# hieucnm/GNN-RecSys

Measured on AMD Instinct MI355X. Metric: edges aggregated/sec, full-graph embed pass, d=128, higher is better.
Workload: dtype fp32

## Files before the change

### gnn-recsys_amd/csrc/spmm_project.hip

```cpp
#include "common.hpp"
#include "gather.hpp"
#include "rowq.hpp"
#include <cstdlib>
#include <type_traits>

namespace gnnrec {
namespace {

constexpr int kPD = 128;
constexpr int kPWaves = 16;
constexpr int kPRows = 2;
constexpr int kFusedChunk = 8;

struct EpiArgs {
  bool relu, l2, attn;
  int accum;
  float out_div, a0, a1;
  float* attn_state;
  float* out;
  int64_t ldo;
  int j0;
};

__device__ __forceinline__ void epilogue_row(const EpiArgs& e, int64_t row, bool valid,
                                             float y0, float y1) {
  activate(e.relu, e.l2, y0, y1);
  float keep = 0.f, nrm_attn = 1.f;
  if (e.attn) {
    float sc = y0 * e.a0 + y1 * e.a1;
#pragma unroll
    for (int off = 1; off < 64; off <<= 1) sc += __shfl_xor(sc, off);
    float mnew = sc, snew = 1.f, cnew = 1.f;
    if (valid && e.accum != GNNREC_ACC_ATTN_FIRST) {
      const float2 st = reinterpret_cast<const float2*>(e.attn_state)[row];
      mnew = fmaxf(st.x, sc);
      keep = expf(st.x - mnew);
      cnew = expf(sc - mnew);
      snew = st.y * keep + cnew;
    }
    if (e.accum == GNNREC_ACC_ATTN_LAST) nrm_attn = 1.f / snew;
    if (valid && (threadIdx.x & 63) == 0)
      reinterpret_cast<float2*>(e.attn_state)[row] = make_float2(mnew, snew);
    y0 *= cnew;
    y1 *= cnew;
  }
  if (!valid) return;
  float2* p = reinterpret_cast<float2*>(e.out + row * e.ldo + e.j0);
  if (e.attn) {
    if (e.accum != GNNREC_ACC_ATTN_FIRST) {
      const float2 o = *p;
      y0 = o.x * keep + y0;
      y1 = o.y * keep + y1;
    }
    y0 *= nrm_attn;
    y1 *= nrm_attn;
  } else if (e.accum != GNNREC_ACC_STORE) {
    const float2 o = *p;
    if (e.accum == GNNREC_ACC_ADD) {
      y0 = o.x + y0;
      y1 = o.y + y1;
    } else {
      y0 = fmaxf(o.x, y0);
      y1 = fmaxf(o.y, y1);
    }
  }
  if (e.out_div > 0.f) {
    y0 = y0 / e.out_div;
    y1 = y1 / e.out_div;
  }
  st_stream2(reinterpret_cast<float*>(p), y0, y1);
}

constexpr int kAggNone = GNNREC_AGG_NONE, kAggSave = GNNREC_AGG_SAVE, kAggLoad = GNNREC_AGG_LOAD;

template <int REDUCE, bool WEIGHTED, int UNROLL, int AGG = kAggNone>
__global__ __launch_bounds__(kPWaves * 64) void spmm_project_kernel(
    const int64_t* __restrict__ indptr, const int32_t* __restrict__ indices,
    const float* __restrict__ ew, const float* __restrict__ X, int64_t ldx,
    const float* __restrict__ H, int64_t ldh, const float* __restrict__ WsT,
    const float* __restrict__ WnT, const float* __restrict__ bias,
    const float* __restrict__ bias_ne, int64_t n_dst, int epilogue, int accum, float out_div,
    const float* __restrict__ attn_vec, float* __restrict__ attn_state,
    float* __restrict__ out, int64_t ldo, unsigned* rq, int rq_ch, float* __restrict__ agg,
    int64_t lda) {
  __shared__ float Ws[kPD * kPD];
  __shared__ float Wn[kPD * kPD];
  __shared__ float slots[kPWaves][kPRows][2][kPD];
  for (int i = threadIdx.x; i < kPD * kPD / 4; i += kPWaves * 64) {
    reinterpret_cast<float4*>(Ws)[i] = reinterpret_cast<const float4*>(WsT)[i];
    reinterpret_cast<float4*>(Wn)[i] = reinterpret_cast<const float4*>(WnT)[i];
  }
  __syncthreads();

  constexpr int LPR = 32, VEC = 4;
  const int lane = threadIdx.x & 63, wave = threadIdx.x >> 6;
  const int grp = lane / LPR;
  const int col = (lane % LPR) * VEC;
  const int j0 = 2 * lane;
  const bool relu = epilogue & GNNREC_EPI_RELU;
  const bool l2 = epilogue & GNNREC_EPI_L2NORM;
  const float init = (REDUCE == GNNREC_REDUCE_MAX) ? -INFINITY : 0.f;
  const int64_t stride = (int64_t)gridDim.x * kPWaves * kPRows;
  const float b0 = bias ? bias[j0] : 0.f, b1 = bias ? bias[j0 + 1] : 0.f;
  const float c0 = bias_ne ? bias_ne[j0] : 0.f, c1 = bias_ne ? bias_ne[j0 + 1] : 0.f;
  const bool attn = accum >= GNNREC_ACC_ATTN_FIRST;
  const float a0 = attn ? attn_vec[j0] : 0.f, a1 = attn ? attn_vec[j0 + 1] : 0.f;
  const EpiArgs ep{relu, l2, attn, accum, out_div, a0, a1, attn_state, out, ldo, j0};

  auto step = [&](int64_t row0, int64_t lim) {
    bool nonempty[kPRows];
    const int nv = (int)(lim - row0 < kPRows ? lim - row0 : kPRows);
    const int64_t ipl = lane <= nv ? ld_stream(indptr + row0 + lane) : 0;
    int64_t rb[kPRows + 1];
#pragma unroll
    for (int r = 0; r <= kPRows; ++r) rb[r] = __shfl(ipl, r <= nv ? r : nv);
    int pidx[kPRows];
    float4 hsr[kPRows];
#pragma unroll
    for (int r = 0; r < kPRows; ++r) {
      const bool valid = r < nv;
      hsr[r] = make_float4(0.f, 0.f, 0.f, 0.f);
      if constexpr (AGG == kAggLoad) {
        pidx[r] = 0;
        if (valid) hsr[r] = ld_stream4((grp == 0 ? agg + (row0 + r) * lda
                                                 : H + (row0 + r) * ldh) + col);
      } else {
        pidx[r] = valid && lane < rb[r + 1] - rb[r] ? ld_stream(indices + rb[r] + lane) : 0;
        if (valid && grp == 1) hsr[r] = ld_stream4(H + (row0 + r) * ldh + col);
      }
    }
#pragma unroll
    for (int r = 0; r < kPRows; ++r) {
      const bool valid = r < nv;
      const float4 hs = hsr[r];
      if constexpr (AGG == kAggLoad) {
        nonempty[r] = rb[r + 1] - rb[r] > 0;
        *reinterpret_cast<float4*>(&slots[wave][r][grp][col]) = hs;
        continue;
      }
      Frag<VEC> acc;
#pragma unroll
      for (int v = 0; v < VEC; ++v) acc.v[v] = init;
      int64_t deg = 0;
      if (valid) {
        const int64_t beg = rb[r], end = rb[r + 1];
        deg = end - beg;
        gather_range<LPR, VEC, REDUCE, WEIGHTED, UNROLL, true>(beg, end, indices, ew, X, ldx,
                                                               col, true, lane, grp, acc, pidx[r]);
      }
      combine_groups<LPR, VEC, REDUCE>(acc);
      finalize<VEC, REDUCE>(acc, deg, 0);
      nonempty[r] = deg > 0;
      if (grp == 0) {
        *reinterpret_cast<float4*>(&slots[wave][r][0][col]) =
            make_float4(acc.v[0], acc.v[1], acc.v[2], acc.v[3]);
        if constexpr (AGG == kAggSave)
          if (valid) store_frag<VEC>(agg + (row0 + r) * lda + col, acc);
      } else {
        *reinterpret_cast<float4*>(&slots[wave][r][1][col]) = hs;
      }
    }
    asm volatile("s_waitcnt lgkmcnt(0)" ::: "memory");

    float z[kPRows][2];
#pragma unroll
    for (int r = 0; r < kPRows; ++r) {
      z[r][0] = b0 + (nonempty[r] ? c0 : 0.f);
      z[r][1] = b1 + (nonempty[r] ? c1 : 0.f);
    }
#pragma unroll 2
    for (int k = 0; k < kPD; k += 4) {
      float4 a4[kPRows], s4[kPRows];
#pragma unroll
      for (int r = 0; r < kPRows; ++r) {
        a4[r] = *reinterpret_cast<const float4*>(&slots[wave][r][0][k]);
        s4[r] = *reinterpret_cast<const float4*>(&slots[wave][r][1][k]);
      }
#pragma unroll
      for (int kk = 0; kk < 4; ++kk) {
        const float2 ws = *reinterpret_cast<const float2*>(&Ws[(k + kk) * kPD + j0]);
        const float2 wn = *reinterpret_cast<const float2*>(&Wn[(k + kk) * kPD + j0]);
#pragma unroll
        for (int r = 0; r < kPRows; ++r) {
          const float s = kk == 0 ? s4[r].x : kk == 1 ? s4[r].y : kk == 2 ? s4[r].z : s4[r].w;
          const float a = kk == 0 ? a4[r].x : kk == 1 ? a4[r].y : kk == 2 ? a4[r].z : a4[r].w;
          z[r][0] = fmaf(s, ws.x, z[r][0]);
          z[r][0] = fmaf(a, wn.x, z[r][0]);
          z[r][1] = fmaf(s, ws.y, z[r][1]);
          z[r][1] = fmaf(a, wn.y, z[r][1]);
        }
      }
    }
    asm volatile("s_waitcnt lgkmcnt(0)" ::: "memory");

#pragma unroll
    for (int r = 0; r < kPRows; ++r) epilogue_row(ep, row0 + r, row0 + r < lim, z[r][0], z[r][1]);
  };

  if (rq != nullptr) {
    rq_for_each(rq, n_dst, rq_ch, [&](int64_t r0, int64_t r1) {
      for (int64_t row0 = r0; row0 < r1; row0 += kPRows) step(row0, r1);
    });
    rq_finish(rq);
    return;
  }
  for (int64_t row0 = ((int64_t)blockIdx.x * kPWaves + wave) * kPRows; row0 < n_dst;
       row0 += stride)
    step(row0, n_dst);
}


constexpr int kSppU = 4;
constexpr int kSpmU = 4;
constexpr int kSpmLU = 2;
constexpr int kSpmEU = 4;
constexpr int kMT = 32;
constexpr int kMWaves = 8;
constexpr int kMRows = kMT / kMWaves;
constexpr int kALd = 2 * kPD + 4;
constexpr int kCLd = kPD + 8;
constexpr int kALds = kMT * kALd;
static_assert(kMRows == 4, "a wave gathers its rows with one gather_lockstep4");

template <int REDUCE, bool WEIGHTED, int UNROLL, bool PRE>
__global__ __launch_bounds__(kMWaves * 64, 4) void spmm_project_mfma_kernel(
    const int64_t* __restrict__ indptr, const int32_t* __restrict__ indices,
    const float* __restrict__ ew, const float* __restrict__ X, int64_t ldx,
    const float* __restrict__ H, int64_t ldh, const float* __restrict__ WsT,
    const float* __restrict__ WnT, const float* __restrict__ bias,
    const float* __restrict__ bias_ne, int64_t n_dst, int epilogue, int accum, float out_div,
    const float* __restrict__ attn_vec, float* __restrict__ attn_state,
    float* __restrict__ out, int64_t ldo, unsigned* rq, int rq_ch) {
  __shared__ float lds[kALds + 2 * kMT * kCLd];
  __shared__ int nes[kMT];
  __shared__ int64_t blk_r[2];
  float* const As = lds;
  float* const Cs0 = lds + kALds;
  float* const Cs1 = Cs0 + kMT * kCLd;

  const int lane = threadIdx.x & 63, wave = threadIdx.x >> 6;
  const int li = lane & 31, bh = lane >> 5;
  const int col = li * 4;
  const int j0 = 2 * lane;
  const int cb = wave & 3, kh = wave >> 2;
  const bool attn = accum >= GNNREC_ACC_ATTN_FIRST;
  const float a0 = attn ? attn_vec[j0] : 0.f, a1 = attn ? attn_vec[j0 + 1] : 0.f;
  const EpiArgs ep{(epilogue & GNNREC_EPI_RELU) != 0, (epilogue & GNNREC_EPI_L2NORM) != 0,
                   attn, accum, out_div, a0, a1, attn_state, out, ldo, j0};

  constexpr int kKL = PRE ? 32 : 64;
  const auto wrsrc = weight_rsrc((kh && !PRE) ? WnT : WsT, kPD * kPD * 4);
  const int wvoff = ((PRE ? 64 * kh + 32 * bh : 64 * bh) * kPD + 32 * cb + li) * 4;

  auto tile = [&](int64_t t0, int64_t lim) __attribute__((always_inline)) {
    const int64_t rbase = t0 + wave * kMRows;
    const int64_t left = lim - rbase;
    const int nv = (int)(left <= 0 ? 0 : left < kMRows ? left : kMRows);
    Frag<4> acc[kMRows];
    int dg[kMRows];
    gather_lockstep4<REDUCE, WEIGHTED, kSpmLU, UNROLL>(indptr, indices, ew, X, ldx, rbase, nv,
                                                       lane, acc, dg);
#pragma unroll
    for (int r = 0; r < kMRows; ++r) {
      const int rl = wave * kMRows + r;
      if (bh == 0)
        *reinterpret_cast<float4*>(&As[rl * kALd + kPD + col]) =
            make_float4(acc[r].v[0], acc[r].v[1], acc[r].v[2], acc[r].v[3]);
      if (lane == 0) nes[rl] = dg[r] > 0;
    }
#pragma unroll
    for (int q = 0; q < kMRows / 2; ++q) {
      const int rl = 2 * q + bh;
      *reinterpret_cast<float4*>(&As[(wave * kMRows + rl) * kALd + col]) =
          rl < nv ? *reinterpret_cast<const float4*>(H + (rbase + rl) * ldh + col)
                  : make_float4(0.f, 0.f, 0.f, 0.f);
    }
    __syncthreads();

    const f32x16 c = mfma_project32<kKL, kPD>(
        wrsrc, wvoff, As + li * kALd + (PRE ? 64 * kh + 32 * bh : kh * kPD + 64 * bh));
    store_c32((kh ? Cs1 : Cs0) + 32 * cb + li, kCLd, bh, c);
    __syncthreads();

#pragma unroll kSpmEU
    for (int r = 0; r < kMRows; ++r) {
      const int rl = wave * kMRows + r;
      const float2 s2 = *reinterpret_cast<const float2*>(&Cs0[rl * kCLd + j0]);
      const float2 n2 = *reinterpret_cast<const float2*>(&Cs1[rl * kCLd + j0]);
      float z0 = s2.x + n2.x, z1 = s2.y + n2.y;
      if constexpr (PRE) {
        const float2 g2 = *reinterpret_cast<const float2*>(&As[rl * kALd + kPD + j0]);
        z0 += g2.x;
        z1 += g2.y;
      }
      if (bias) {
        z0 = bias[j0] + z0;
        z1 = bias[j0 + 1] + z1;
      }
      if (bias_ne && nes[rl]) {
        z0 = bias_ne[j0] + z0;
        z1 = bias_ne[j0 + 1] + z1;
      }
      epilogue_row(ep, rbase + r, r < nv, z0, z1);
    }
    __syncthreads();
  };

  TileCursor<kMT> cur;
  cur.begin(rq, n_dst, rq_ch, blk_r);
  int64_t r0, r1;
  while (cur.next(r0, r1))
    for (int64_t t0 = r0; t0 < r1; t0 += kMT) tile(t0, r1);
  if (rq != nullptr) rq_finish(rq);
}

}
}

using namespace gnnrec;

static int launch_spmm_project(const char* name, const int64_t* indptr, const int32_t* indices,
                               const float* ew, const float* X, int64_t ldx, const float* H,
                               int64_t ldh, const float* W_selfT, const float* W_neighT,
                               const float* bias, const float* bias_nonempty, int64_t n_dst,
                               int64_t d, int reduce, int epilogue, int accum, float out_div,
                               const float* attn_vec, float* attn_state, float* out, int64_t ldo,
                               float* agg, int64_t lda, int agg_mode, void* stream) {
  GNNREC_REQUIRE(reduce == GNNREC_REDUCE_SUM || reduce == GNNREC_REDUCE_MEAN ||
                     reduce == GNNREC_REDUCE_MAX,
                 "%s: unknown reduce %d", name, reduce);
  GNNREC_REQUIRE(agg_mode == GNNREC_AGG_NONE || agg_mode == GNNREC_AGG_SAVE ||
                     agg_mode == GNNREC_AGG_LOAD,
                 "%s: unknown aggregate mode %d", name, agg_mode);
  const bool load = agg_mode == GNNREC_AGG_LOAD;
  const int st = load ? fused_check(name, d, epilogue, false, accum, attn_vec, attn_state, n_dst,
                                    'X', {indptr, H, W_selfT}, {H, W_selfT, W_neighT}, {ldh}, out,
                                    ldo)
                      : fused_check(name, d, epilogue, false, accum, attn_vec, attn_state, n_dst,
                                    'X', {indptr, X, H, W_selfT}, {X, H, W_selfT, W_neighT},
                                    {ldx, ldh}, out, ldo);
  if (st != GNNREC_OK || n_dst == 0) return st;
  GNNREC_REQUIRE(W_neighT, "%s: W_neighT = NULL (pre-projected source "
                           "rows) is gnnrec_spmm_project_mfma_f32's form", name);
  if (agg_mode != GNNREC_AGG_NONE) {
    GNNREC_REQUIRE(agg, "%s: the aggregate mode needs agg", name);
    GNNREC_REQUIRE(aligned16(agg) && lda >= kPD && lda % 4 == 0,
                   "%s: agg needs 16-B aligned rows of lda >= %d floats", name, kPD);
  }
  const int64_t per_block = (int64_t)kPWaves * kPRows;
  const int64_t blocks = persistent_blocks((n_dst + per_block - 1) / per_block, 1);
  const int rq_ch = kFusedChunk;
  hipStream_t s = as_stream(stream);
  int ticket = -1;
  unsigned* rq = rowq_slot_for(n_dst, blocks * kPWaves, rq_ch, s, &ticket);
  const dim3 grid((unsigned)blocks), block(kPWaves * 64);
  auto launch = [&](auto r, auto w, auto m) {
    hipLaunchKernelGGL(
        (spmm_project_kernel<decltype(r)::value, decltype(w)::value, kSppU, decltype(m)::value>),
        grid, block, 0, s, indptr, indices, ew, X, ldx, H, ldh, W_selfT, W_neighT, bias,
        bias_nonempty, n_dst, epilogue, accum, out_div, attn_vec, attn_state, out, ldo, rq, rq_ch,
        agg, lda);
  };
  using Sum = std::integral_constant<int, GNNREC_REDUCE_SUM>;
  if (load) {
    launch(Sum{}, std::false_type{}, std::integral_constant<int, kAggLoad>{});
  } else {
    dispatch_bool(ew != nullptr, [&](auto w) {
      dispatch_reduce(reduce, [&](auto r) {
        if (agg_mode == GNNREC_AGG_SAVE)
          launch(r, w, std::integral_constant<int, kAggSave>{});
        else
          launch(r, w, std::integral_constant<int, kAggNone>{});
      });
    });
  }
  rowq_launched(ticket, s);
  return check_launch(name);
}

extern "C" int gnnrec_spmm_project_f32(const int64_t* indptr, const int32_t* indices,
                                       const float* ew, const float* X, int64_t ldx,
                                       const float* H, int64_t ldh, const float* W_selfT,
                                       const float* W_neighT, const float* bias,
                                       const float* bias_nonempty, int64_t n_dst, int64_t d,
                                       int reduce, int epilogue, int accum, float out_div,
                                       const float* attn_vec, float* attn_state, float* out,
                                       int64_t ldo, void* stream) {
  return launch_spmm_project("gnnrec_spmm_project_f32", indptr, indices, ew, X, ldx, H, ldh,
                             W_selfT, W_neighT, bias, bias_nonempty, n_dst, d, reduce, epilogue,
                             accum, out_div, attn_vec, attn_state, out, ldo, nullptr, 0,
                             GNNREC_AGG_NONE, stream);
}

extern "C" int gnnrec_spmm_project_agg_f32(const int64_t* indptr, const int32_t* indices,
                                           const float* ew, const float* X, int64_t ldx,
                                           const float* H, int64_t ldh, const float* W_selfT,
                                           const float* W_neighT, const float* bias,
                                           const float* bias_nonempty, int64_t n_dst, int64_t d,
                                           int reduce, int epilogue, int accum, float out_div,
                                           const float* attn_vec, float* attn_state, float* out,
                                           int64_t ldo, float* agg, int64_t lda, int agg_mode,
                                           void* stream) {
  return launch_spmm_project("gnnrec_spmm_project_agg_f32", indptr, indices, ew, X, ldx, H, ldh,
                             W_selfT, W_neighT, bias, bias_nonempty, n_dst, d, reduce, epilogue,
                             accum, out_div, attn_vec, attn_state, out, ldo, agg, lda, agg_mode,
                             stream);
}

extern "C" int gnnrec_spmm_project_mfma_f32(const int64_t* indptr, const int32_t* indices,
                                            const float* ew, const float* X, int64_t ldx,
                                            const float* H, int64_t ldh, const float* W_selfT,
                                            const float* W_neighT, const float* bias,
                                            const float* bias_nonempty, int64_t n_dst,
                                            int64_t d, int reduce, int epilogue, int accum,
                                            float out_div, const float* attn_vec,
                                            float* attn_state, float* out, int64_t ldo,
                                            void* stream) {
  const char* const name = "gnnrec_spmm_project_mfma_f32";
  GNNREC_REQUIRE(reduce == GNNREC_REDUCE_SUM || reduce == GNNREC_REDUCE_MEAN ||
                     reduce == GNNREC_REDUCE_MAX,
                 "gnnrec_spmm_project_mfma_f32: unknown reduce %d", reduce);
  const int st = fused_check(name, d, epilogue, false, accum, attn_vec, attn_state, n_dst, 'X',
                             {indptr, X, H, W_selfT}, {X, H, W_selfT, W_neighT}, {ldx, ldh}, out,
                             ldo);
  if (st != GNNREC_OK || n_dst == 0) return st;
  const bool pre = W_neighT == nullptr;
  GNNREC_REQUIRE(!pre || reduce != GNNREC_REDUCE_MAX,
                 "gnnrec_spmm_project_mfma_f32: pre-projected rows (W_neighT = NULL) need a "
                 "sum or mean reduce");
  const int64_t blocks = persistent_blocks((n_dst + kMT - 1) / kMT, 2);
  constexpr int rq_ch = 2 * kMT;
  hipStream_t s = as_stream(stream);
  int ticket = -1;
  unsigned* rq = rowq_slot_for(n_dst, blocks, rq_ch, s, &ticket);
  const dim3 grid((unsigned)blocks), block(kMWaves * 64);
  dispatch_bool(pre, [&](auto p) {
    dispatch_bool(ew != nullptr, [&](auto w) {
      dispatch_reduce(reduce, [&](auto r) {
        constexpr int R = decltype(r)::value;
        constexpr bool P = decltype(p)::value;
        if constexpr (!(P && R == GNNREC_REDUCE_MAX))
          hipLaunchKernelGGL((spmm_project_mfma_kernel<R, decltype(w)::value, kSpmU, P>), grid,
                             block, 0, s, indptr, indices, ew, X, ldx, H, ldh, W_selfT, W_neighT,
                             bias, bias_nonempty, n_dst, epilogue, accum, out_div, attn_vec,
                             attn_state, out, ldo, rq, rq_ch);
      });
    });
  });
  rowq_launched(ticket, s);
  return check_launch(name);
}

namespace gnnrec {
namespace {

constexpr int kP2Waves = 16;
constexpr int kP2U = 5;

struct PreRel {
  const int64_t* indptr;
  const int32_t* indices;
  const float* ew;
  const float* Y;
  int64_t ldy;
  const float* bias_ne;
  int mean;
};

constexpr int kP2Win = 48;

__device__ __forceinline__ void dma4(const int32_t* src, int32_t* lds) {
#if defined(__HIP_DEVICE_COMPILE__)
  __builtin_amdgcn_global_load_lds(src, (__attribute__((address_space(3))) void*)lds, 4, 0, 0);
#endif
}

struct PairWalk {
  RqCursor c;
  int64_t pos, c1;
  bool queued;
};

__device__ __forceinline__ bool walk_next(PairWalk& w, unsigned* rq, int64_t n_dst, int rq_ch,
                                          int64_t stride, int64_t& row0, int64_t& lim) {
  if (!w.queued) {
    if (w.pos >= n_dst) return false;
    row0 = w.pos;
    lim = n_dst;
    w.pos += stride;
    return true;
  }
  if (w.pos >= w.c1) {
    int64_t r0, r1;
    if (!rq_next(w.c, rq, n_dst, rq_ch, r0, r1)) return false;
    w.pos = r0;
    w.c1 = r1;
  }
  row0 = w.pos;
  lim = w.c1;
  w.pos += kPRows;
  return true;
}

template <bool WA, bool WB, int NT = 0>
__global__ __launch_bounds__(kP2Waves * 64) void spmm_project2_pipe_kernel(
    PreRel ra, PreRel rb, const float* __restrict__ H, int64_t ldh,
    const float* __restrict__ WaT, const float* __restrict__ WbT,
    const float* __restrict__ bias_a, const float* __restrict__ bias_b, int64_t n_dst,
    int epilogue, int combine, const float* __restrict__ attn_vec, float out_div,
    float* __restrict__ out, int64_t ldo, unsigned* rq, int rq_ch) {
  __shared__ float Wa[kPD * kPD];
  __shared__ float Wb[kPD * kPD];
  __shared__ float slots[kP2Waves][kPRows][kPD];
  __shared__ int32_t win[kP2Waves][2][kPRows][kP2Win];
  __shared__ int64_t bnd[kP2Waves][2][kPRows + 1];
  for (int i = threadIdx.x; i < kPD * kPD / 4; i += kP2Waves * 64) {
    reinterpret_cast<float4*>(Wa)[i] = reinterpret_cast<const float4*>(WaT)[i];
    reinterpret_cast<float4*>(Wb)[i] = reinterpret_cast<const float4*>(WbT)[i];
  }
  __syncthreads();

  constexpr int LPR = 32, VEC = 4, U = kP2U, NPI = kWave / LPR;
  const int lane = threadIdx.x & 63, wave = threadIdx.x >> 6;
  const int grp = lane / LPR;
  const int col = (lane % LPR) * VEC;
  const int j0 = 2 * lane;
  const bool relu = epilogue & GNNREC_EPI_RELU;
  const bool l2 = epilogue & GNNREC_EPI_L2NORM;
  const int64_t stride = (int64_t)gridDim.x * kP2Waves * kPRows;
  const float ba0 = bias_a ? bias_a[j0] : 0.f, ba1 = bias_a ? bias_a[j0 + 1] : 0.f;
  const float bb0 = bias_b ? bias_b[j0] : 0.f, bb1 = bias_b ? bias_b[j0 + 1] : 0.f;
  const float ca0 = ra.bias_ne ? ra.bias_ne[j0] : 0.f, ca1 = ra.bias_ne ? ra.bias_ne[j0 + 1] : 0.f;
  const float cb0 = rb.bias_ne ? rb.bias_ne[j0] : 0.f, cb1 = rb.bias_ne ? rb.bias_ne[j0 + 1] : 0.f;
  const float at0 = attn_vec ? attn_vec[j0] : 0.f, at1 = attn_vec ? attn_vec[j0 + 1] : 0.f;

  auto load_bounds = [&](int64_t row0, int nv) __attribute__((always_inline)) {
    const int l = lane & 31;
    const int64_t* ip = lane < 32 ? ra.indptr : rb.indptr;
    return l <= nv ? ld_stream(ip + row0 + l) : (int64_t)0;
  };
  auto stage_heads = [&](int64_t bv, int nv) __attribute__((always_inline)) {
    int64_t ba[kPRows + 1], bb[kPRows + 1];
#pragma unroll
    for (int i = 0; i <= kPRows; ++i) {
      ba[i] = __shfl(bv, i <= nv ? i : nv);
      bb[i] = __shfl(bv, 32 + (i <= nv ? i : nv));
    }
    if (lane <= kPRows) {
      bnd[wave][0][lane] = ba[lane <= nv ? lane : nv];
      bnd[wave][1][lane] = bb[lane <= nv ? lane : nv];
    }
#pragma unroll
    for (int i = 0; i < kPRows; ++i) {
      if (i < nv) {
        if (lane < ba[i + 1] - ba[i] && lane < kP2Win)
          dma4(ra.indices + ba[i] + lane, &win[wave][0][i][0]);
        if (lane < bb[i + 1] - bb[i] && lane < kP2Win)
          dma4(rb.indices + bb[i] + lane, &win[wave][1][i][0]);
      }
    }
  };
  auto gather_row = [&](const PreRel& r, auto weighted, auto nt, int64_t beg, int64_t end,
                        int pre_idx, Frag<VEC>& acc) __attribute__((always_inline)) {
    constexpr bool W = decltype(weighted)::value;
    constexpr bool NTR = decltype(nt)::value;
    int64_t base = beg;
    int wlen = kP2Win;
    while (base < end) {
      const int cnt = (int)((end - base) < wlen ? (end - base) : wlen);
      const int myidx = base == beg ? pre_idx : (lane < cnt ? ld_stream(r.indices + base + lane) : 0);
      float myw = 0.f;
      if constexpr (W) myw = lane < cnt ? ld_stream(r.ew + base + lane) : 0.f;
      for (int j = 0; j < cnt; j += NPI * U) {
        Frag<VEC> val[U];
        bool ok[U];
#pragma unroll
        for (int u = 0; u < U; ++u) {
          const int k = j + u * NPI + grp;
          ok[u] = k < cnt;
          const int src = edge_bcast<NPI>(myidx, j + u * NPI, grp);
          if (ok[u]) {
            if constexpr (NTR) {
              const float4 t = ld_stream4(r.Y + (int64_t)src * r.ldy + col);
              val[u].v[0] = t.x; val[u].v[1] = t.y; val[u].v[2] = t.z; val[u].v[3] = t.w;
            } else {
              load_frag<VEC>(val[u], r.Y + (int64_t)src * r.ldy + col);
            }
          } else {
#pragma unroll
            for (int v = 0; v < VEC; ++v) val[u].v[v] = 0.f;
          }
        }
#pragma unroll
        for (int u = 0; u < U; ++u) {
          float w = 1.f;
          if constexpr (W) w = edge_bcast<NPI>(myw, j + u * NPI, grp);
#pragma unroll
          for (int v = 0; v < VEC; ++v) acc.v[v] += W ? val[u].v[v] * w : val[u].v[v];
        }
      }
      base += wlen;
      wlen = 64;
    }
  };
  auto finish_rel = [&](const PreRel& r, Frag<VEC>& acc, int64_t deg, float (&g)[2])
      __attribute__((always_inline)) {
    combine_groups<LPR, VEC, GNNREC_REDUCE_SUM>(acc);
    if (r.mean) finalize<VEC, GNNREC_REDUCE_MEAN>(acc, deg, 0);
    const int sl = lane >> 1;
    const float x0 = __shfl(acc.v[0], sl), x1 = __shfl(acc.v[1], sl);
    const float x2 = __shfl(acc.v[2], sl), x3 = __shfl(acc.v[3], sl);
    g[0] = (lane & 1) ? x2 : x0;
    g[1] = (lane & 1) ? x3 : x1;
  };

  PairWalk walk;
  walk.queued = rq != nullptr;
  walk.pos = ((int64_t)blockIdx.x * kP2Waves + wave) * kPRows;
  walk.c1 = 0;
  if (walk.queued) rq_begin(walk.c, rq);
  int64_t row0, lim;
  bool have = walk_next(walk, rq, n_dst, rq_ch, stride, row0, lim);
  if (have) {
    const int nv = (int)(lim - row0 < kPRows ? lim - row0 : kPRows);
    stage_heads(load_bounds(row0, nv), nv);
  }
  while (have) {
    asm volatile("s_waitcnt vmcnt(0) lgkmcnt(0)" ::: "memory");
    const int nv = (int)(lim - row0 < kPRows ? lim - row0 : kPRows);
    int64_t rba[kPRows + 1], rbb[kPRows + 1];
    int pa[kPRows], pb[kPRows];
#pragma unroll
    for (int i = 0; i <= kPRows; ++i) {
      rba[i] = bnd[wave][0][i];
      rbb[i] = bnd[wave][1][i];
    }
#pragma unroll
    for (int i = 0; i < kPRows; ++i) {
      pa[i] = lane < kP2Win ? win[wave][0][i][lane] : 0;
      pb[i] = lane < kP2Win ? win[wave][1][i][lane] : 0;
    }
    int64_t nrow0 = 0, nlim = 0;
    const bool next = walk_next(walk, rq, n_dst, rq_ch, stride, nrow0, nlim);
    const int nnv = next ? (int)(nlim - nrow0 < kPRows ? nlim - nrow0 : kPRows) : 0;
    const int64_t nbv = next ? load_bounds(nrow0, nnv) : 0;
#pragma unroll
    for (int i = 0; i < kPRows; ++i) {
      const float4 hs = i < nv && grp == 0 ? ld_stream4(H + (row0 + i) * ldh + col)
                                           : make_float4(0.f, 0.f, 0.f, 0.f);
      if (grp == 0) *reinterpret_cast<float4*>(&slots[wave][i][col]) = hs;
    }
    float ga[kPRows][2], gb[kPRows][2];
    bool nea[kPRows], neb[kPRows];
#pragma unroll
    for (int i = 0; i < kPRows; ++i) {
      Frag<VEC> acc;
#pragma unroll
      for (int v = 0; v < VEC; ++v) acc.v[v] = 0.f;
      const int64_t deg = i < nv ? rba[i + 1] - rba[i] : 0;
      if (i < nv)
        gather_row(ra, std::integral_constant<bool, WA>{}, std::integral_constant<bool, NT == 1>{},
                   rba[i], rba[i + 1], pa[i], acc);
      finish_rel(ra, acc, deg, ga[i]);
      nea[i] = deg > 0;
    }
    asm volatile("s_waitcnt lgkmcnt(0)" ::: "memory");
    if (next) stage_heads(nbv, nnv);
#pragma unroll
    for (int i = 0; i < kPRows; ++i) {
      Frag<VEC> acc;
#pragma unroll
      for (int v = 0; v < VEC; ++v) acc.v[v] = 0.f;
      const int64_t deg = i < nv ? rbb[i + 1] - rbb[i] : 0;
      if (i < nv)
        gather_row(rb, std::integral_constant<bool, WB>{}, std::integral_constant<bool, NT == 2>{},
                   rbb[i], rbb[i + 1], pb[i], acc);
      finish_rel(rb, acc, deg, gb[i]);
      neb[i] = deg > 0;
    }
    asm volatile("s_waitcnt lgkmcnt(0)" ::: "memory");

    float za[kPRows][2], zb[kPRows][2];
#pragma unroll
    for (int i = 0; i < kPRows; ++i) {
      za[i][0] = ba0 + (nea[i] ? ca0 : 0.f);
      za[i][1] = ba1 + (nea[i] ? ca1 : 0.f);
      zb[i][0] = bb0 + (neb[i] ? cb0 : 0.f);
      zb[i][1] = bb1 + (neb[i] ? cb1 : 0.f);
    }
#pragma unroll 2
    for (int k = 0; k < kPD; k += 4) {
      float4 s4[kPRows];
#pragma unroll
      for (int i = 0; i < kPRows; ++i) s4[i] = *reinterpret_cast<const float4*>(&slots[wave][i][k]);
#pragma unroll
      for (int kk = 0; kk < 4; ++kk) {
        const float2 wa = *reinterpret_cast<const float2*>(&Wa[(k + kk) * kPD + j0]);
        const float2 wb = *reinterpret_cast<const float2*>(&Wb[(k + kk) * kPD + j0]);
#pragma unroll
        for (int i = 0; i < kPRows; ++i) {
          const float sv = kk == 0 ? s4[i].x : kk == 1 ? s4[i].y : kk == 2 ? s4[i].z : s4[i].w;
          za[i][0] = fmaf(sv, wa.x, za[i][0]);
          za[i][1] = fmaf(sv, wa.y, za[i][1]);
          zb[i][0] = fmaf(sv, wb.x, zb[i][0]);
          zb[i][1] = fmaf(sv, wb.y, zb[i][1]);
        }
      }
    }
    asm volatile("s_waitcnt lgkmcnt(0)" ::: "memory");

#pragma unroll
    for (int i = 0; i < kPRows; ++i) {
      float ya0 = za[i][0] + ga[i][0], ya1 = za[i][1] + ga[i][1];
      float yb0 = zb[i][0] + gb[i][0], yb1 = zb[i][1] + gb[i][1];
      activate(relu, l2, ya0, ya1);
      activate(relu, l2, yb0, yb1);
      combine2_store(ya0, ya1, yb0, yb1, combine, at0, at1, out_div, i < nv,
                     out + (row0 + i) * ldo + j0);
    }
    row0 = nrow0;
    lim = nlim;
    have = next;
  }
  if (rq != nullptr) rq_finish(rq);
}

}
}

extern "C" int gnnrec_spmm_project2_f32(
    const int64_t* indptr_a, const int32_t* indices_a, const float* ew_a, const float* Ya,
    int64_t ldya, int reduce_a, const float* bias_nonempty_a, const int64_t* indptr_b,
    const int32_t* indices_b, const float* ew_b, const float* Yb, int64_t ldyb, int reduce_b,
    const float* bias_nonempty_b, const float* H, int64_t ldh, const float* W_self_aT,
    const float* W_self_bT, const float* bias_a, const float* bias_b, int64_t n_dst, int64_t d,
    int epilogue, int combine, const float* attn_vec, float out_div, float* out, int64_t ldo,
    void* stream) {
  const char* const name = "gnnrec_spmm_project2_f32";
  int nt = ((reduce_a & GNNREC_SRC_STREAM) ? 1 : 0) | ((reduce_b & GNNREC_SRC_STREAM) ? 2 : 0);
  if (nt == 3) nt = 0;
  reduce_a &= ~GNNREC_SRC_STREAM;
  reduce_b &= ~GNNREC_SRC_STREAM;
  GNNREC_REQUIRE((reduce_a == GNNREC_REDUCE_SUM || reduce_a == GNNREC_REDUCE_MEAN) &&
                     (reduce_b == GNNREC_REDUCE_SUM || reduce_b == GNNREC_REDUCE_MEAN),
                 "gnnrec_spmm_project2_f32: pre-projected relations reduce by sum or mean");
  const int st = fused_check(name, d, epilogue, true, combine, attn_vec, nullptr, n_dst, 'Y',
                             {indptr_a, Ya, indptr_b, Yb, H, W_self_aT, W_self_bT},
                             {Ya, Yb, H, W_self_aT, W_self_bT}, {ldya, ldyb, ldh}, out, ldo);
  if (st != GNNREC_OK || n_dst == 0) return st;
  const int64_t per_block = (int64_t)kP2Waves * kPRows;
  const int64_t blocks = persistent_blocks((n_dst + per_block - 1) / per_block, 1);
  constexpr int rq_ch = 16;
  hipStream_t s = as_stream(stream);
  int ticket = -1;
  unsigned* rq = rowq_slot_for(n_dst, blocks * kP2Waves, rq_ch, s, &ticket);
  const dim3 grid((unsigned)blocks), block(kP2Waves * 64);
  const PreRel a{indptr_a, indices_a, ew_a, Ya, ldya, bias_nonempty_a,
                 reduce_a == GNNREC_REDUCE_MEAN};
  const PreRel b{indptr_b, indices_b, ew_b, Yb, ldyb, bias_nonempty_b,
                 reduce_b == GNNREC_REDUCE_MEAN};
  auto launch = [&](auto wa, auto wb, auto ntc) {
    hipLaunchKernelGGL(
        (spmm_project2_pipe_kernel<decltype(wa)::value, decltype(wb)::value, decltype(ntc)::value>),
        grid, block, 0, s, a, b, H, ldh, W_self_aT, W_self_bT, bias_a, bias_b, n_dst, epilogue,
        combine, attn_vec, out_div, out, ldo, rq, rq_ch);
  };
  dispatch_bool(ew_a != nullptr, [&](auto wa) {
    dispatch_bool(ew_b != nullptr, [&](auto wb) {
      using NT0 = std::integral_constant<int, 0>;
      if constexpr (!decltype(wa)::value && !decltype(wb)::value) {
        if (nt == 1) launch(wa, wb, std::integral_constant<int, 1>{});
        else if (nt == 2) launch(wa, wb, std::integral_constant<int, 2>{});
        else launch(wa, wb, NT0{});
      } else {
        launch(wa, wb, NT0{});
      }
    });
  });
  rowq_launched(ticket, s);
  return check_launch(name);
}
```

Before: 24.92 billion.

## Add MFMA kernel for the aggregate-load projection path with async LDS staging

```diff
diff --git a/gnn-recsys_amd/csrc/spmm_project.hip b/gnn-recsys_amd/csrc/spmm_project.hip
--- a/gnn-recsys_amd/csrc/spmm_project.hip
+++ b/gnn-recsys_amd/csrc/spmm_project.hip
@@ -71,7 +71,7 @@
   st_stream2(reinterpret_cast<float*>(p), y0, y1);
 }
 
-constexpr int kAggNone = GNNREC_AGG_NONE, kAggSave = GNNREC_AGG_SAVE, kAggLoad = GNNREC_AGG_LOAD;
+constexpr int kAggNone = GNNREC_AGG_NONE, kAggSave = GNNREC_AGG_SAVE;
 
 template <int REDUCE, bool WEIGHTED, int UNROLL, int AGG = kAggNone>
 __global__ __launch_bounds__(kPWaves * 64) void spmm_project_kernel(
@@ -120,24 +120,13 @@
     for (int r = 0; r < kPRows; ++r) {
       const bool valid = r < nv;
       hsr[r] = make_float4(0.f, 0.f, 0.f, 0.f);
-      if constexpr (AGG == kAggLoad) {
-        pidx[r] = 0;
-        if (valid) hsr[r] = ld_stream4((grp == 0 ? agg + (row0 + r) * lda
-                                                 : H + (row0 + r) * ldh) + col);
-      } else {
-        pidx[r] = valid && lane < rb[r + 1] - rb[r] ? ld_stream(indices + rb[r] + lane) : 0;
-        if (valid && grp == 1) hsr[r] = ld_stream4(H + (row0 + r) * ldh + col);
-      }
+      pidx[r] = valid && lane < rb[r + 1] - rb[r] ? ld_stream(indices + rb[r] + lane) : 0;
+      if (valid && grp == 1) hsr[r] = ld_stream4(H + (row0 + r) * ldh + col);
     }
 #pragma unroll
     for (int r = 0; r < kPRows; ++r) {
       const bool valid = r < nv;
       const float4 hs = hsr[r];
-      if constexpr (AGG == kAggLoad) {
-        nonempty[r] = rb[r + 1] - rb[r] > 0;
-        *reinterpret_cast<float4*>(&slots[wave][r][grp][col]) = hs;
-        continue;
-      }
       Frag<VEC> acc;
 #pragma unroll
       for (int v = 0; v < VEC; ++v) acc.v[v] = init;
@@ -311,6 +300,145 @@
   int64_t r0, r1;
   while (cur.next(r0, r1))
     for (int64_t t0 = r0; t0 < r1; t0 += kMT) tile(t0, r1);
+  if (rq != nullptr) rq_finish(rq);
+}
+
+
+constexpr int kLWaves = 4;
+constexpr int kLRows = kMT / kLWaves;
+static_assert(kMT * kCLd <= kALds, "the C tile lives in the A buffer the MFMAs have consumed");
+
+__device__ __forceinline__ void dma16(const float* src, float* lds) {
+#if defined(__HIP_DEVICE_COMPILE__)
+  __builtin_amdgcn_global_load_lds(src, (__attribute__((address_space(3))) void*)lds, 16, 0, 2);
+#endif
+}
+
+__global__ __launch_bounds__(kLWaves * 64, 2) void spmm_project_load_mfma_kernel(
+    const int64_t* __restrict__ indptr, const float* __restrict__ H, int64_t ldh,
+    const float* __restrict__ agg, int64_t lda, const float* __restrict__ WsT,
+    const float* __restrict__ WnT, const float* __restrict__ bias,
+    const float* __restrict__ bias_ne, int64_t n_dst, int epilogue, int accum, float out_div,
+    const float* __restrict__ attn_vec, float* __restrict__ attn_state,
+    float* __restrict__ out, int64_t ldo, unsigned* rq, int rq_ch) {
+  __shared__ __attribute__((aligned(16))) float As[2][kALds];
+  __shared__ int nes[2][kMT];
+  __shared__ int64_t blk_r[2];
+
+  const int lane = threadIdx.x & 63, wave = __builtin_amdgcn_readfirstlane(threadIdx.x >> 6);
+  const int li = lane & 31, bh = lane >> 5;
+  const int col = li * 4;
+  const int j0 = 2 * lane;
+  const int cj = 32 * wave + li;
+  const bool attn = accum >= GNNREC_ACC_ATTN_FIRST;
+  const float a0 = attn ? attn_vec[j0] : 0.f, a1 = attn ? attn_vec[j0 + 1] : 0.f;
+  const EpiArgs ep{(epilogue & GNNREC_EPI_RELU) != 0, (epilogue & GNNREC_EPI_L2NORM) != 0,
+                   attn, accum, out_div, a0, a1, attn_state, out, ldo, j0};
+  const float bj = bias ? bias[cj] : 0.f, cjn = bias_ne ? bias_ne[cj] : 0.f;
+
+  float bw[kPD];
+  {
+    const float* wp = (bh ? WnT : WsT) + cj;
+#pragma unroll
+    for (int k = 0; k < kPD; ++k) bw[k] = wp[k * kPD];
+  }
+
+  int64_t ip0 = 0, ip1 = 0;
+  auto request = [&](int b, int64_t t0, int64_t lim) __attribute__((always_inline)) {
+    ip0 = ip1 = 0;
+    if (threadIdx.x < kMT) {
+      const int64_t row = t0 + threadIdx.x;
+      if (row < lim) {
+        ip0 = ld_stream(indptr + row);
+        ip1 = ld_stream(indptr + row + 1);
+      }
+    }
+#pragma unroll
+    for (int r = 0; r < kLRows; ++r) {
+      const int rl = wave * kLRows + r;
+      const int64_t row = t0 + rl;
+      if (row < lim) dma16((bh ? agg + row * lda : H + row * ldh) + col, &As[b][rl * kALd]);
+    }
+  };
+
+  auto uniform = [](int64_t v) __attribute__((always_inline)) {
+    return (int64_t)(((uint64_t)(unsigned)__builtin_amdgcn_readfirstlane((int)(v >> 32)) << 32) |
+                     (unsigned)__builtin_amdgcn_readfirstlane((int)v));
+  };
+  TileCursor<kMT> cur;
+  cur.begin(rq, n_dst, rq_ch, blk_r);
+  int64_t t0, lim;
+  bool have = cur.next(t0, lim);
+  t0 = uniform(t0);
+  lim = uniform(lim);
+  if (have) request(0, t0, lim);
+  int buf = 0;
+  while (have) {
+    asm volatile("s_waitcnt vmcnt(0)" ::: "memory");
+    if (threadIdx.x < kMT) nes[buf][threadIdx.x] = ip1 - ip0 > 0;
+    int64_t nt0 = 0, nlim = 0;
+    const bool more = cur.next(nt0, nlim);
+    nt0 = uniform(nt0);
+    nlim = uniform(nlim);
+
+    f32x16 c;
+#pragma unroll
+    for (int v = 0; v < 16; ++v)
+      c[v] = bj + (nes[buf][(v & 3) + 8 * (v >> 2) + 4 * bh] ? cjn : 0.f);
+    __builtin_amdgcn_sched_barrier(0);
+    if (more) request(buf ^ 1, nt0, nlim);
+    __builtin_amdgcn_sched_barrier(0);
+
+    const unsigned ap = (unsigned)(uintptr_t)(
+        __attribute__((address_space(3))) const float*)&As[buf][li * kALd + bh * kPD];
+    constexpr int kAC = 16;
+    f32x4s a[2][kAC / 4];
+    auto read_a = [&](int ch) __attribute__((always_inline)) {
+      asm volatile("ds_read_b128 %0, %4\n\t"
+                   "ds_read_b128 %1, %4 offset:16\n\t"
+                   "ds_read_b128 %2, %4 offset:32\n\t"
+                   "ds_read_b128 %3, %4 offset:48"
+                   : "=&v"(a[ch & 1][0]), "=&v"(a[ch & 1][1]), "=&v"(a[ch & 1][2]),
+                     "=&v"(a[ch & 1][3])
+                   : "v"(ap + ch * kAC * 4)
+                   : "memory");
+    };
+    auto landed_a = [&](int ch) __attribute__((always_inline)) {
+      asm volatile("s_waitcnt lgkmcnt(0)"
+                   : "+v"(a[ch & 1][0]), "+v"(a[ch & 1][1]), "+v"(a[ch & 1][2]),
+                     "+v"(a[ch & 1][3])
+                   :
+                   : "memory");
+    };
+    read_a(0);
+#pragma unroll
+    for (int ch = 0; ch < kPD / kAC; ++ch) {
+      landed_a(ch);
+      if (ch + 1 < kPD / kAC) read_a(ch + 1);
+      __builtin_amdgcn_sched_barrier(0);
+#pragma unroll
+      for (int i = 0; i < kAC; ++i)
+        c = __builtin_amdgcn_mfma_f32_32x32x2f32(a[ch & 1][i / 4][i % 4], bw[ch * kAC + i], c, 0,
+                                                 0, 0);
+      __builtin_amdgcn_sched_barrier(0);
+    }
+    __syncthreads();
+
+    float* const Cs = As[buf];
+    store_c32(Cs + cj, kCLd, bh, c);
+    __syncthreads();
+
+#pragma unroll kSpmEU
+    for (int r = 0; r < kLRows; ++r) {
+      const int rl = wave * kLRows + r;
+      const float2 z = *reinterpret_cast<const float2*>(&Cs[rl * kCLd + j0]);
+      epilogue_row(ep, t0 + rl, t0 + rl < lim, z.x, z.y);
+    }
+    t0 = nt0;
+    lim = nlim;
+    have = more;
+    buf ^= 1;
+  }
   if (rq != nullptr) rq_finish(rq);
 }
 
@@ -347,11 +475,22 @@
     GNNREC_REQUIRE(aligned16(agg) && lda >= kPD && lda % 4 == 0,
                    "%s: agg needs 16-B aligned rows of lda >= %d floats", name, kPD);
   }
+  hipStream_t s = as_stream(stream);
+  int ticket = -1;
+  if (load) {
+    const int64_t blocks = persistent_blocks((n_dst + kMT - 1) / kMT, 2);
+    constexpr int rq_ch = kMT;
+    unsigned* rq = rowq_slot_for(n_dst, blocks, rq_ch, s, &ticket);
+    hipLaunchKernelGGL(spmm_project_load_mfma_kernel, dim3((unsigned)blocks),
+                       dim3(kLWaves * 64), 0, s, indptr, H, ldh, agg, lda, W_selfT, W_neighT,
+                       bias, bias_nonempty, n_dst, epilogue, accum, out_div, attn_vec,
+                       attn_state, out, ldo, rq, rq_ch);
+    rowq_launched(ticket, s);
+    return check_launch(name);
+  }
   const int64_t per_block = (int64_t)kPWaves * kPRows;
   const int64_t blocks = persistent_blocks((n_dst + per_block - 1) / per_block, 1);
   const int rq_ch = kFusedChunk;
-  hipStream_t s = as_stream(stream);
-  int ticket = -1;
   unsigned* rq = rowq_slot_for(n_dst, blocks * kPWaves, rq_ch, s, &ticket);
   const dim3 grid((unsigned)blocks), block(kPWaves * 64);
   auto launch = [&](auto r, auto w, auto m) {
@@ -361,19 +500,14 @@
         bias_nonempty, n_dst, epilogue, accum, out_div, attn_vec, attn_state, out, ldo, rq, rq_ch,
         agg, lda);
   };
-  using Sum = std::integral_constant<int, GNNREC_REDUCE_SUM>;
-  if (load) {
-    launch(Sum{}, std::false_type{}, std::integral_constant<int, kAggLoad>{});
-  } else {
-    dispatch_bool(ew != nullptr, [&](auto w) {
-      dispatch_reduce(reduce, [&](auto r) {
-        if (agg_mode == GNNREC_AGG_SAVE)
-          launch(r, w, std::integral_constant<int, kAggSave>{});
-        else
-          launch(r, w, std::integral_constant<int, kAggNone>{});
-      });
+  dispatch_bool(ew != nullptr, [&](auto w) {
+    dispatch_reduce(reduce, [&](auto r) {
+      if (agg_mode == GNNREC_AGG_SAVE)
+        launch(r, w, std::integral_constant<int, kAggSave>{});
+      else
+        launch(r, w, std::integral_constant<int, kAggNone>{});
     });
-  }
+  });
   rowq_launched(ticket, s);
   return check_launch(name);
 }
```

Result: faster. 26.93 billion (median of 6 runs) (+8.1%).
